# famoreno/stereo-vo

Hardware: AMD Instinct MI355X
Metric: stereo pairs/sec @1280×960 (higher is better)
Workload: dtype u8/f64

## Files before the change

### stereo_vo_amd/csrc/k_detect.hip

```cpp
#include <algorithm>
#include "svo_device.h"
#include "svo_kernels.h"
#include "faster_dyn.hpp"
#include "../../include/svo_orb_tables.h"

__constant__ int c_umax[16];
__device__ __attribute__((aligned(16))) float4 g_brief_patf[SVO_BRIEF_NPAIRS];
__device__ __attribute__((aligned(16))) uint4 g_blur_gh[3 * 64], g_blur_gv[3 * 64];
#define SVO_DISC_E 256
__device__ uint32_t g_disc_m[SVO_DISC_E], g_disc_x[SVO_DISC_E];
#define DP_REACH SVO_BRIEF_REACH
#define DP_BW (2 * DP_REACH + 1)
#define DP_RW (DP_BW + 6)
#define DP_X0 (DP_REACH + 5)

hipError_t svo_upload_tables()
{
    hipError_t e = hipMemcpyToSymbol(HIP_SYMBOL(c_umax), svo_umax, sizeof(svo_umax));
    if (e != hipSuccess) return e;
    {
        static float4 pf[SVO_BRIEF_NPAIRS];
        for (int i = 0; i < SVO_BRIEF_NPAIRS; i++) pf[i] = make_float4((float)svo_brief_pat[i][0], (float)svo_brief_pat[i][2], (float)svo_brief_pat[i][1], (float)svo_brief_pat[i][3]);
        e = hipMemcpyToSymbol(HIP_SYMBOL(g_brief_patf), pf, sizeof(pf));
        if (e != hipSuccess) return e;
// ... 829 lines not shown
    return a;
}

__device__ __forceinline__ void sincos_f32(float x, float& sn, float& cs)
{
    const int k = (int)(x * 0.63661977f + 0.5f);
    const float fk = (float)k;
    const float r = ((x - fk * 1.5703125f) - fk * 4.837512969970703125e-4f) - fk * 7.54978995489188216e-8f;
    const float z = r * r;
    const float sp = ((-1.9515295891e-4f * z + 8.3321608736e-3f) * z - 1.6666654611e-1f) * z * r + r;
    const float cp = ((2.443315711809948e-5f * z - 1.388731625493765e-3f) * z + 4.166664568298827e-2f) * z * z - 0.5f * z + 1.0f;
    const bool odd = k & 1;
    const float s0 = odd ? cp : sp, c0 = odd ? sp : cp;
    sn = (k & 2) ? -s0 : s0;
    cs = (((k + 1) & 2) != 0) ? -c0 : c0;
}

__device__ __forceinline__ uint32_t udot4(uint32_t a, uint32_t b, uint32_t acc)
{
    return __builtin_amdgcn_udot4(a, b, acc, false);
}

template <int NW, bool TL>
__global__ void __launch_bounds__(NW * 64) k_describe(DevCtx c, FastDiv gx_div, int pre, int kpw)
{
    SVO_TL_SCOPE(c, TL_DESCRIBE, pre);
    __shared__ __attribute__((aligned(16))) uint32_t raw32[NW][2][DP_LROWS * DP_PW + 4];
    __shared__ __attribute__((aligned(16))) float4 s_pat[SVO_BRIEF_NPAIRS];
    __shared__ uint32_t s_disc_m[SVO_DISC_E], s_disc_x[SVO_DISC_E];
    static_assert(NW * 64 == SVO_BRIEF_NPAIRS && NW * 64 == SVO_DISC_E, "one table entry per thread");
    __shared__ __attribute__((aligned(16))) uint4 s_gh[TL ? 3 * 64 : 1], s_gv[TL ? 3 * 64 : 1];
    if (c.idle.w[0] | c.idle.w[1]) {
        const int img_b = c.debug_mode == DBG_LINEAR_TILES ? (int)(blockIdx.x / gx_div.d) : (int)(fastdiv(blockIdx.x >> 3, gx_div) * 8 + (blockIdx.x & 7));
        if (img_b < c.n_img && lane_idle(c, img_b >> 1)) return;
    }
    s_pat[threadIdx.x] = g_brief_patf[threadIdx.x]; s_disc_m[threadIdx.x] = g_disc_m[threadIdx.x]; s_disc_x[threadIdx.x] = g_disc_x[threadIdx.x];
    if (TL && threadIdx.x < 3 * 64) { s_gh[threadIdx.x] = g_blur_gh[threadIdx.x]; s_gv[threadIdx.x] = g_blur_gv[threadIdx.x]; }
    __syncthreads();
    const int wid = __builtin_amdgcn_readfirstlane((int)(threadIdx.x >> 6)), lane = threadIdx.x & 63;
    int img, bx;
    if (c.debug_mode == DBG_LINEAR_TILES) { img = blockIdx.x / gx_div.d; bx = blockIdx.x - img * gx_div.d; }
    else { const uint32_t r = blockIdx.x >> 3, grp = fastdiv(r, gx_div); bx = (int)(r - grp * gx_div.d); img = (int)(grp * 8 + (blockIdx.x & 7)); }
    if (img >= c.n_img) return;
    const int lane_id = img >> 1, vl0 = lane_id * c.oct_cap;
    const int n_end = __builtin_amdgcn_readfirstlane(pre ? c.desc_n[img] : c.n_slots);
    const int slot0 = (bx * NW + wid) * kpw;
    if (slot0 >= n_end) return;
    const int slot1 = min(slot0 + kpw, n_end);
    const long long fo0 = pre ? feat_base(c, vl0, 1 - c.lane[lane_id].prev_slot, img & 1) : 0;
    dp_v4i GH[3], GV[3];
#pragma unroll
    for (int t = 0; t < 3; t++) { if (!TL) { GH[t] = *(const dp_v4i*)&g_blur_gh[t * 64 + lane]; GV[t] = *(const dp_v4i*)&g_blur_gv[t * 64 + lane]; } else { GH[t] = dp_v4i{0, 0, 0, 0}; GV[t] = GH[t]; } }
#pragma unroll
    for (int t = 0; t < 3; t++) if (!TL) asm volatile("" : "+v"(GH[t]), "+v"(GV[t]));
    uint32_t w_pos = 0, w_lvl = 0;
    if (slot0 + lane < slot1) {
        if (pre) { const uint2 w = c.desc_work[(long long)img * c.raw_cap + slot0 + lane]; w_pos = w.x; w_lvl = w.y; }
        else w_pos = c.lvl_pos[(long long)img * c.raw_cap + slot0 + lane];
    }
    asm volatile("" : "+v"(w_pos), "+v"(w_lvl));
    auto item = [&](int slot, int& live, int& x, int& y, int& level) {
        const uint32_t pos = (uint32_t)__builtin_amdgcn_readlane((int)w_pos, slot - slot0);
        int lv = 0, ok = 1;
        if (pre) lv = __builtin_amdgcn_readlane((int)w_lvl, slot - slot0);
        else {
#pragma unroll
            for (int l = 1; l < SVO_MAX_LEVELS; l++) if (l < c.n_levels && slot >= c.lv[l].slot_off) lv = l;
            lv = __builtin_amdgcn_readfirstlane(lv);
            ok = __builtin_amdgcn_readfirstlane(slot - c.lv[lv].slot_off < c.lvl_n[img * SVO_MAX_LEVELS + lv] ? 1 : 0);
        }
        level = lv; live = ok; x = (int)(pos & 0xFFFFu); y = (int)(pos >> 16);
    };
    const uint8_t* base0; const uint8_t* pyr0 = c.pyr + (long long)img * c.pyr_bytes;
    {
        const uint64_t b = (uint64_t)(uintptr_t)c.img0[img];
        base0 = (const uint8_t*)(uintptr_t)(((uint64_t)(uint32_t)__builtin_amdgcn_readfirstlane((int)(b >> 32)) << 32) | (uint32_t)__builtin_amdgcn_readfirstlane((int)(uint32_t)b));
    }
    const int cr0 = (lane * 171) >> 9, cq0 = lane - 3 * cr0, cr1 = ((lane + 64) * 171) >> 9, cq1 = lane + 64 - 3 * cr1;
    auto stage = [&](uint32_t* dst, int x, int y, int level) {
        const int pitch = level == 0 ? c.img0_pitch : c.lv[level].pitch;
        const uint8_t* lim = level == 0 ? base0 : pyr0 + c.lv[level].offset;
        const uint8_t* org = lim + (uint32_t)((y - (DP_REACH + 3)) * pitch + (x - DP_X0));
        const uint32_t lb = (uint32_t)__builtin_amdgcn_readfirstlane((int)(uint32_t)(uintptr_t)(__attribute__((address_space(3))) uint32_t*)dst);
        glds16_asm(org + (uint32_t)(cr0 * pitch + 16 * cq0), lb);
        glds16_asm(org + (uint32_t)(cr1 * pitch + 16 * cq1), lb + 1024);
        if (lane < DP_RW * 3 - 128) glds16_asm(org + (uint32_t)(42 * pitch + 32), lb + 2048);
    };
    static_assert(DP_RW * 3 - 128 == 1, "the third DMA instruction carries chunk 128 alone");
    int live, x, y, level;
    item(slot0, live, x, y, level);
    if (live) stage(raw32[wid][0], x, y, level);
    const int n16 = lane & 15, q4 = lane >> 4;
    for (int slot = slot0; slot < slot1; slot++) {
        uint32_t* R32 = raw32[wid][(slot - slot0) & 1];
        int live_n = 0, x_n = 0, y_n = 0, level_n = 0;
        if (slot + 1 < slot1) item(slot + 1, live_n, x_n, y_n, level_n);
        live_n = __builtin_amdgcn_readfirstlane(live_n); x_n = __builtin_amdgcn_readfirstlane(x_n); y_n = __builtin_amdgcn_readfirstlane(y_n); level_n = __builtin_amdgcn_readfirstlane(level_n);
        asm volatile("s_waitcnt vmcnt(0)" ::: "memory");
        wave_lds_sync();
        if (live_n) stage(raw32[wid][(slot - slot0 + 1) & 1], x_n, y_n, level_n);
        if (live) {
            uint32_t m10u = 0; int m01 = 0, msum = 0;
#pragma unroll
            for (int i = 0; i < 4; i++) {
                const int en = i * 64 + lane;
                const int vr = en >> 3, d = en & 7;
                const uint32_t px = R32[(vr + 6) * DP_PW + 2 + d];
                const uint32_t s = udot4(px, s_disc_m[en], 0u);
                m10u = udot4(px, s_disc_x[en], m10u);
                msum += (int)s;
                m01 += __mul24(vr - 15, (int)s);
            }
            const int m10 = wave_sum_uniform((int)m10u - 15 * msum);
            m01 = wave_sum_uniform(m01);
            float angle, sn, cs;
            if (c.debug_mode == DBG_DESCRIBE_NO_TRIG) { angle = (float)(m10 & 255); sn = (float)(m01 & 255) * 0.001f; cs = 1.f - sn; }
            else { angle = atan2_deg((float)m01, (float)m10); sincos_f32(angle * 0.017453292f, sn, cs); }
            dp_v4i S[3][3];
            {
                if (TL) {
#pragma unroll
                    for (int t = 0; t < 3; t++) GH[t] = *(const dp_v4i*)&s_gh[t * 64 + lane];
                }
// ... 38 lines not shown
                        asm("v_sat_pk_u8_i16 %0, %1" : "=v"(s23) : "v"(h23));
                        *(uint32_t*)&Bl[(16 * ot + n16) * (4 * DP_PW) + 16 * nt + 4 * q4] = __builtin_amdgcn_perm(s23, s01, 0x05040100u);
                    }
                }
            }
            wave_lds_sync();
            const float MX = 12582912.0f + (float)(DP_REACH + (int)((uint8_t*)R32 - (uint8_t*)&raw32[0][0][0])), MY = 12582912.0f + (float)DP_REACH;
            const uint8_t* lds0 = (const uint8_t*)&raw32[0][0][0];
            unsigned long long bits[4];
            typedef float dp_f2 __attribute__((ext_vector_type(2)));
            const dp_f2 cs2 = { cs, cs }, sn2 = { sn, sn }, MX2 = { MX, MX }, MY2 = { MY, MY };
#pragma unroll
            for (int k = 0; k < 4; k++) {
                const float4 pt = s_pat[k * 64 + lane];
                const dp_f2 px = { pt.x, pt.y }, py = { pt.z, pt.w };
                const dp_f2 xs = (px * cs2 - py * sn2) + MX2, ys = (px * sn2 + py * cs2) + MY2;
                const uint32_t o0 = (__umul24(__float_as_uint(ys.x), 4 * DP_PW) + __float_as_uint(xs.x)) & 0xFFFFu;
                const uint32_t o1 = (__umul24(__float_as_uint(ys.y), 4 * DP_PW) + __float_as_uint(xs.y)) & 0xFFFFu;
                const int a = lds0[o0], b = lds0[o1];
                bits[k] = __ballot(a < b);
            }
            if (lane == 0) {
                if (pre) {
                    const long long fo = fo0 + slot;
                    unsigned long long* d = (unsigned long long*)(c.desc + fo * 32);
                    d[0] = bits[0]; d[1] = bits[1]; d[2] = bits[2]; d[3] = bits[3];
                    c.kps[fo].angle = angle;
                } else {
                    const LevelGeom& g = c.lv[level];
                    const long long o = (long long)img * c.raw_cap + slot;
                    unsigned long long* d = (unsigned long long*)(c.raw_desc + o * 32);
                    d[0] = bits[0]; d[1] = bits[1]; d[2] = bits[2]; d[3] = bits[3];
                    svo_keypoint k;
                    k.x = (float)x * g.scale; k.y = (float)y * g.scale; k.size = c.fast_orb ? 7.0f : 31.0f * g.scale; k.angle = angle;
                    k.response = c.lvl_resp[o]; k.octave = c.fast_orb ? 0 : level; k.class_id = -1;
                    c.raw_kps[o] = k;
                }
            }
        }
        live = live_n; x = x_n; y = y_n; level = level_n;
    }
}

typedef unsigned long long sad_row_t __attribute__((aligned(1)));
template <bool ANY_SLOT>
__device__ __forceinline__ void sad_patch_body(const DevCtx& c, int which)
{
    const int vs = blockIdx.y, vl = vs >> 1, side = vs & 1, lane_id = vl / c.oct_cap, oct = vl % c.oct_cap;
    if (oct >= c.n_oct || lane_idle(c, lane_id)) return;
    const int prev = c.lane[lane_id].prev_slot;
    const int cur = (ANY_SLOT && which) ? prev : 1 - prev;
    const int n = c.n_kps[feat_cnt_idx(vl, cur, side)];
    const int i = blockIdx.x * 32 + (threadIdx.x >> 3), r = threadIdx.x & 7;
    if (i >= n) return;
    const long long fo = feat_base(c, vl, cur, side) + i;
    const svo_keypoint k = c.kps[fo];
    const int W = c.ow[oct], H = c.oh[oct];
    const bool border = k.x < 3.0f || k.y < 3.0f || k.x > (float)(W - 5) || k.y > (float)(H - 5);
    if (ANY_SLOT && (k.x != k.x || k.y != k.y)) { if (r == 0) c.sad_flag[fo] = 1; return; }
    if (r == 0) c.sad_flag[fo] = border ? 1 : 0;
    if (border) return;
    int pitch;
    const uint8_t* img = level_ptr(c, lane_id * 2 + side, c.fast_orb ? oct : 0, pitch);
// ... 1100 lines not shown
    if (c.n_tiles <= 0) return;
    const long long total = (long long)c.n_tiles * c.n_img, unit = 8 * FT_CHUNK;
    hipLaunchKernelGGL(k_fast, dim3((unsigned)((total + unit - 1) / unit * unit)), dim3(FT_NT), 0, st, c);
}

template <class F> static auto select_form(int sel_max, F f)
{
    if (sel_max > 4096) return f(std::integral_constant<int, 8192>());
    if (sel_max > 2048) return f(std::integral_constant<int, 4096>());
    return f(std::integral_constant<int, 2048>());
}

void launch_select(const DevCtx& c, hipStream_t st)
{
    const dim3 grid(c.n_img, c.n_levels);
    auto select = [&](int pass) { select_form(c.sel_max, [&](auto s) { hipLaunchKernelGGL(k_select<decltype(s)::value>, grid, dim3(512), 0, st, c, pass); }); };
    select(0);
    hipLaunchKernelGGL(k_fast_redo, dim3(4096), dim3(FT_NT), 0, st, c);
    select(1);
    hipLaunchKernelGGL(k_harris, dim3(c.n_img, c.sel_max / 256, c.n_levels), dim3(256), 0, st, c);
    select_form(c.sel_max, [&](auto s) { constexpr int S = decltype(s)::value; hipLaunchKernelGGL(k_select_sort<S>, grid, dim3(512), (size_t)LdsSelectSort<S>{}.total(), st, c); });
}

void launch_describe(const DevCtx& c, const Knobs& k, int pre, hipStream_t st)
{
    if (c.n_slots <= 0) return;
    const int kpw = k.desc_kpw, per = 4 * kpw, gx = (c.n_slots + per - 1) / per, img8 = (c.n_img + 7) / 8 * 8;
    if (k.desc_tl) hipLaunchKernelGGL((k_describe<4, true>), dim3((unsigned)((long long)gx * img8)), dim3(256), 0, st, c, make_fastdiv((uint32_t)gx), (pre && !c.fast_orb) ? 1 : 0, kpw);
    else hipLaunchKernelGGL((k_describe<4, false>), dim3((unsigned)((long long)gx * img8)), dim3(256), 0, st, c, make_fastdiv((uint32_t)gx), (pre && !c.fast_orb) ? 1 : 0, kpw);
}

void launch_sad_patch(const DevCtx& c, hipStream_t st)
{
    const int n = c.fast_orb ? c.max_kps : std::min(c.n_slots, c.max_kps);
    if (n <= 0) return;
    hipLaunchKernelGGL(k_sad_patch, dim3((n + 31) / 32, c.n_lanes * c.oct_cap * 2), dim3(256), 0, st, c);
}

void launch_publish_img0(const DevCtx& c, const uint8_t* const* ptrs, hipStream_t st)
{
    ImgPtrs ip;
    for (int i = 0; i < 2 * SVO_MAX_LANES; i++) ip.p[i] = i < c.n_img ? ptrs[i] : nullptr;
    hipLaunchKernelGGL(k_publish_img0, dim3((c.n_img + 255) / 256), dim3(256), 0, st, c, ip);
}
void launch_sad_patch_slot(const DevCtx& c, int which, hipStream_t st)
{
    hipLaunchKernelGGL(k_sad_patch_slot, dim3((c.max_kps + 31) / 32, c.n_lanes * c.oct_cap * 2), dim3(256), 0, st, c, which);
}

template <class T> static LdsChunkedNms<typename T::Key> chunked_nms_layout(const DevCtx& c) { return {FO_PMAX, c.max_kps}; }
static int nms_pmax(const DevCtx& c)
{
// ... 102 lines not shown
```

### stereo_vo_amd/csrc/svo_api.hip

```cpp
#include "svo_device.h"
#include "svo_kernels.h"
#include "state_format.hpp"
#include "frame_call.hpp"
#include "lk_call.hpp"
#include "gftt_call.hpp"
#include "klt_call.hpp"
#include <math.h>
#include <string.h>
#include <stdio.h>
#include <stdlib.h>
#include <string>
#include <vector>
#include <mutex>
#include <map>
#include <memory>
#include <condition_variable>

#define HIPCHECK(expr) do { hipError_t _e = (expr); if (_e != hipSuccess) { ctx->last_error = std::string(#expr) + ": " + hipGetErrorString(_e); return SVO_ERR_HIP; } } while (0)

enum { KT_BEGIN, KT_RESIZE, KT_FAST, KT_SELECT, KT_DESCRIBE, KT_NMS, KT_HAM_LR, KT_LR_FILTER, KT_HAM_TRK, KT_TRK_FILTER,
       KT_RANSAC_HYP, KT_RANSAC_CNT, KT_TRK_FINAL, KT_GN, KT_RANSAC_HYP1, KT_RANSAC_CNT1, KT_RANSAC_HYP2, KT_RANSAC_CNT2,
       KT_SAD_PATCH, KT_LR_SAD, KT_TRK_SAD,
       KT_SELECT_8192, KT_NMS_16, KT_HAM_LR_WIDE, KT_HAM_TRK_WIDE, KT_TRK_FILTER_64,
       KT_EXPORT, KT_IMPORT, KT_EXPORT_WIN, KT_IMPORT_WIN,
// ... 32 lines not shown
        for (const char* name : { "librocprofiler-sdk-roctx.so.1", "librocprofiler-sdk-roctx.so", "libroctx64.so.4", "libroctx64.so" }) {
            void* h = dlopen(name, RTLD_LAZY | RTLD_GLOBAL);
            if (!h) continue;
            push = (int (*)(const char*))dlsym(h, "roctxRangePushA");
            pop = (int (*)())dlsym(h, "roctxRangePop");
            if (push && pop) return;
            push = nullptr; pop = nullptr;
        }
    }
};
RoctxApi& roctx_api() { static RoctxApi a; return a; }
struct Section {
    bool on;
    explicit Section(const char* name) : on(roctx_api().push != nullptr) { if (on) roctx_api().push(name); }
    ~Section() { if (on) roctx_api().pop(); }
    Section(const Section&) = delete; Section& operator=(const Section&) = delete;
};
}
extern "C" int svo_profiler_sections_enabled(void) { return roctx_api().push != nullptr; }

struct svo_ctx {
    svo_config cfg;
    Knobs knobs;
    svo_params params;
    int fast_th, orb_th;
    int klt_win;
    hipStream_t stream, stream0; bool own_stream;
    DevCtx dc;
    bool geom_ready, geom_once;
    int geom_w, geom_h, geom_nfe, geom_nlevels, geom_method, geom_noct;
    int raw_cap_alloc;
    uint8_t* d_img0; int img0_pitch_internal;
    uint8_t* d_img0_ring[2]; uint8_t* h_stage[2]; size_t slot_bytes;
    hipStream_t s_copy; hipEvent_t ev_h2d[2], ev_det[2]; bool ev_det_valid[2], ev_h2d_valid[2], up_ready; int up_slot, det_slot;
    long long pyr_bytes_alloc; int cand_total_alloc, rtab_alloc, tile_tab_alloc;
    std::vector<void*> allocs;
    std::string last_error;
    std::vector<TimedSpan> spans; std::vector<hipEvent_t> free_events;
    double kt_total[KT_EVERY]; long long kt_calls[KT_EVERY]; unsigned long long kt_mask;
    unsigned* d_ham_out; uint8_t* d_ham_q, *d_ham_t; int ham_cap_q, ham_cap_t;
    uint8_t* d_lk_pyr; size_t lk_pyr_cap; LkJobDev* d_lk_jobs; int lk_jobs_cap;
    float2* d_lk_pts, *d_lk_init, *d_lk_out; uint8_t* d_lk_status; float* d_lk_err; int lk_pts_cap;
    std::vector<LkJobDev> lk_jobs; bool lk_used;
    float* d_gftt_map; size_t gftt_map_cap; uint8_t* d_gftt_img; size_t gftt_img_cap; GfttJobDev* d_gftt_jobs; int gftt_jobs_cap;
    unsigned long long* d_gftt_keys; int* d_gftt_items; uint8_t* d_gftt_state; int* d_gftt_info;
    float2* d_gftt_seeds; int gftt_seeds_cap; float2* d_gftt_pts; float* d_gftt_resp; int gftt_pts_cap;
// ... 267 lines not shown
    ctx->d_lk_pyr = nullptr; ctx->lk_pyr_cap = 0; ctx->d_lk_jobs = nullptr; ctx->lk_jobs_cap = 0; ctx->lk_pts_cap = 0; ctx->lk_used = false;
    ctx->d_lk_pts = ctx->d_lk_init = ctx->d_lk_out = nullptr; ctx->d_lk_status = nullptr; ctx->d_lk_err = nullptr;
    ctx->d_gftt_map = nullptr; ctx->gftt_map_cap = 0; ctx->d_gftt_img = nullptr; ctx->gftt_img_cap = 0; ctx->d_gftt_jobs = nullptr; ctx->gftt_jobs_cap = 0;
    ctx->d_gftt_keys = nullptr; ctx->d_gftt_items = nullptr; ctx->d_gftt_state = nullptr; ctx->d_gftt_info = nullptr;
    ctx->d_gftt_seeds = nullptr; ctx->gftt_seeds_cap = 0; ctx->d_gftt_pts = nullptr; ctx->d_gftt_resp = nullptr; ctx->gftt_pts_cap = 0; ctx->gftt_used = false;
    memset(&ctx->klt, 0, sizeof(ctx->klt)); ctx->params_set = false; ctx->frame_parallel = false; ctx->ransac_feed_used = false;
    ctx->d_src = nullptr; ctx->src_pitch = 0; ctx->d_map_ptrs = nullptr; ctx->map_w = ctx->map_h = ctx->n_maps = 0;
    ctx->map_shared[0] = ctx->map_shared[1] = nullptr; ctx->d_rect_models = nullptr;
    memset(&ctx->imported, 0, sizeof(ctx->imported)); ctx->graph_replays = 0; ctx->capturing = false; ctx->frame_active_set = false; memset(&ctx->frame_active, 0, sizeof(ctx->frame_active)); ctx->use_graphs = false; ctx->d_anms = nullptr; ctx->post_event = nullptr; ctx->pose_cov = false; ctx->d_cov = nullptr; ctx->d_cov_mask = nullptr;
    ctx->landmarks = false; ctx->lmk_std = 1.0; ctx->d_lmk = nullptr; ctx->d_lmk_info = nullptr; ctx->d_lmk_cnt = nullptr;
    ctx->sad.cur.assign((size_t)cfg->n_lanes, 1); ctx->sad.prev.assign((size_t)cfg->n_lanes, 1); ctx->sad.drop.assign((size_t)cfg->n_lanes, 0);
    ctx->cip_ready = false; ctx->d_vals = nullptr; ctx->h_vals = nullptr; ctx->vals_bytes = 0;
    ctx->up_ready = false; ctx->up_slot = 0; ctx->det_slot = -1; ctx->s_copy = nullptr; ctx->slot_bytes = 0;
    for (int i = 0; i < 2; i++) { ctx->d_img0_ring[i] = nullptr; ctx->h_stage[i] = nullptr; ctx->ev_det_valid[i] = ctx->ev_h2d_valid[i] = false; }
    for (int i = 0; i < KT_EVERY; i++) { ctx->kt_total[i] = 0; ctx->kt_calls[i] = 0; }
    ctx->kt_mask = ~0ull;
    *out = ctx;
    knobs_read(&ctx->knobs, knobs_env);
    if (svo_ab_form_requested(ctx->knobs) && !svo_ab_kernels_built()) {
        ctx->last_error = "SVO_HAM_FP4=0 / SVO_DEBUG_MODE=14 / 52 ask for an A/B kernel form that this library was built without: load libsvo_hip_ab.so (SVO_HIP_LIB) or build with -DSVO_AB_KERNELS";
        return SVO_ERR_UNSUPPORTED;
    }
    HIPCHECK(hipSetDevice(cfg->device));
    if (cfg->stream) { ctx->stream = (hipStream_t)cfg->stream; ctx->own_stream = false; }
    else { HIPCHECK(hipStreamCreateWithFlags(&ctx->stream, hipStreamNonBlocking)); ctx->own_stream = true; }
    ctx->stream0 = ctx->stream;
    HIPCHECK(svo_upload_tables());
    DevCtx& d = ctx->dc;
    memset(&d, 0, sizeof(d));
    const int L = cfg->n_lanes, NI = 2 * L, MK = cfg->max_kps;
    const int OC = cfg->max_octaves < 1 ? 1 : (cfg->max_octaves > SVO_MAX_OCTAVES ? SVO_MAX_OCTAVES : cfg->max_octaves);
    const int NV = L * OC;
    d.n_lanes = L; d.n_img = NI; d.max_kps = MK; d.n_levels = SVO_MAX_LEVELS; d.oct_cap = OC; d.n_oct = 1; d.max_h = cfg->max_h;
    ctx->raw_cap_alloc = 2 * MK;
    ctx->pyr_bytes_alloc = pyramid_bytes(cfg->max_w, cfg->max_h, SVO_MAX_LEVELS);
    ctx->cand_total_alloc = (int)((long long)cfg->max_cand * 33 / 10) + 8 * 1024;
    ctx->rtab_alloc = 2 * (cfg->max_w + cfg->max_h) * SVO_MAX_LEVELS;
    ctx->img0_pitch_internal = align_up(cfg->max_w, 64);
    HIPCHECK(dev_alloc(ctx, &ctx->d_img0, (size_t)NI * ctx->img0_pitch_internal * cfg->max_h));
    HIPCHECK(dev_alloc(ctx, (uint8_t***)&d.img0, (size_t)NI));
    HIPCHECK(dev_alloc(ctx, &d.pyr, (size_t)NI * ctx->pyr_bytes_alloc));
    HIPCHECK(dev_alloc(ctx, &d.rtab, (size_t)ctx->rtab_alloc));
    ctx->tile_tab_alloc = 4 * ((cfg->max_w / SVO_FT_W + 2) * (cfg->max_h / SVO_FT_H + 2)) + 64;
    HIPCHECK(dev_alloc(ctx, (uint4**)&d.fast_tiles, (size_t)ctx->tile_tab_alloc));
    HIPCHECK(dev_alloc(ctx, &d.cand_keys, (size_t)NI * ctx->cand_total_alloc));
    HIPCHECK(dev_alloc(ctx, &d.cand_cnt, (size_t)NI * SVO_MAX_LEVELS * SVO_CNT_STRIDE));
// ... 1003 lines not shown
{
    DevCtx& d = ctx->dc; const svo_params& p = ctx->params;
    if (call.faster) {
        { Span s(ctx, KT_RESIZE); for (int l = 1; l < d.n_levels; l++) launch_half(d, l, st); }
        if (call.faster_anms) {
            if (ctx->dyn_fast) { Span s(ctx, KT_FASTER); launch_faster_dyn(d, ctx->d_cand64, ctx->d_fstats, ctx->dyn_target, ctx->klt_win, st); }
            else { Span s(ctx, KT_FASTER); launch_faster(d, ctx->d_cand64, p.initial_FAST_threshold, ctx->klt_win, st); }
            { Span s(ctx, KT_FASTER_NMS); launch_faster_anms(d, ctx->d_cand64, ctx->d_fanms, ctx->dyn_fast ? ctx->d_fstats : nullptr, ctx->dyn_target, st); }
            return;
        }
        if (ctx->dyn_fast) {
            { Span s(ctx, KT_FASTER); launch_faster_dyn(d, ctx->d_cand64, ctx->d_fstats, ctx->dyn_target, ctx->klt_win, st); }
            { Span s(ctx, KT_FASTER_NMS); launch_faster_nms_dyn(d, ctx->d_cand64, p.non_maximal_suppression, p.min_distance, ctx->d_fstats, ctx->dyn_target, st); }
            return;
        }
        { Span s(ctx, KT_FASTER); launch_faster(d, ctx->d_cand64, p.initial_FAST_threshold, ctx->klt_win, st); }
        { Span s(ctx, KT_FASTER_NMS); launch_faster_nms(d, ctx->d_cand64, p.non_maximal_suppression, p.min_distance, st); }
    } else if (d.fast_orb) {
        { Span s(ctx, KT_RESIZE); for (int l = 1; l < d.n_levels; l++) launch_half(d, l, st); }
        { Span s(ctx, KT_FAST); launch_fast(d, st); }
        if (p.non_maximal_suppression && p.nmsMethod == SVO_NMS_ADAPTIVE) {
            Span s(ctx, KT_SELECT); launch_fastorb_anms(d, ctx->d_anms, st);
        } else { Span s(ctx, KT_SELECT); launch_fastorb_nms(d, p.non_maximal_suppression, p.min_distance, st); }
        { Span s(ctx, KT_DESCRIBE); launch_describe(d, ctx->knobs, 0, st); }
    } else {
        { Span s(ctx, KT_RESIZE); for (int l = 1; l < d.n_levels; l++) launch_resize(d, l, st); }
        { Span s(ctx, KT_FAST); launch_fast(d, st); }
        if (!call.select_in_post) { Span s(ctx, kt_select(d)); launch_select(d, st); }
        if (d.debug_mode == DBG_DESCRIBE_BEFORE_NMS) { Span s(ctx, KT_DESCRIBE); launch_describe(d, ctx->knobs, 0, st); }
    }
}
static void enqueue_detect_post(svo_ctx* ctx, const FrameCall& call, hipStream_t st)
{
    DevCtx& d = ctx->dc; const svo_params& p = ctx->params;
    if (call.select_in_post && !d.fast_orb) { Span s(ctx, kt_select(d)); launch_select(d, st); }
    const bool described = d.fast_orb || d.debug_mode == DBG_DESCRIBE_BEFORE_NMS;
    { Span s(ctx, kt_nms(d)); launch_nms_rowsort(d, ctx->knobs, d.fast_orb ? call.nms_mode_oct : call.nms_mode, p.min_distance, described ? 0 : 1, st); }
    if (!described) { Span s(ctx, KT_DESCRIBE); launch_describe(d, ctx->knobs, 1, st); }
}
static void enqueue_match(svo_ctx* ctx, const FrameCall& call, hipStream_t st)
{
    DevCtx& d = ctx->dc; const svo_params& p = ctx->params;
    Section sec("_stg3"), sec2("stg3.find_pairings");
    if (p.match_method == SVO_SM_DESC_BF) {
        { Span s(ctx, wide_lists(d) ? KT_HAM_LR_WIDE : KT_HAM_LR); launch_hamming(d, ctx->knobs, 0, hamming_splits(ctx), st); }
        { Span s(ctx, KT_LR_FILTER); launch_match_lr_filter(d, p.enable_robust_1to1_match, p.max_y_diff, st); }
    } else if (p.match_method == SVO_SM_DESC_RBR) {
        Span s(ctx, KT_LR_FILTER);
        launch_match_lr_rbr(d, false, p.enable_robust_1to1_match, p.max_y_diff, call.minresp, (int)(size_t)p.orb_max_distance, st);
    } else {
        Span s(ctx, KT_LR_SAD);
        launch_match_lr_rbr(d, true, p.enable_robust_1to1_match, p.max_y_diff, call.minresp, call.max_sad_match, st);
    }
}
static void set_ransac_chunks(svo_ctx* ctx)
{
    DevCtx& d = ctx->dc;
    const int forced = ctx->knobs.rs_c0;
    d.rs_c0 = forced ? forced : (d.n_lanes * d.n_oct > 8 ? SVO_RANSAC_CHUNK0 : SVO_RANSAC_FEW);
    d.rs_c1 = d.rs_c0 > SVO_RANSAC_CHUNK1 ? d.rs_c0 : SVO_RANSAC_CHUNK1;
}
// ... 1678 lines not shown
```

### stereo_vo_amd/csrc/svo_kernels.h

```cpp
#pragma once
#include "svo_device.h"
#include "rectify_model.hpp"

struct GNParams {
    int use_robust_kernel, max_iters, initial_max_iters, max_incr_cost;
    int use_previous_pose_as_initial, use_custom_initial_pose;
    int min_distance, img_w, img_h;
    int pmax;
    int standalone;
    int pad;
    double kernel_param, min_mod_out_vector, residual_threshold;
    double init[6];
    uint8_t* mask_out;
};

bool svo_ab_kernels_built();
hipError_t svo_upload_tables();
hipError_t svo_raise_dyn_smem(const void* kernel, size_t bytes);
struct PrepArgs {
    const uint8_t* src[2 * SVO_MAX_LANES];
    const uint2* const* maps;
    uint8_t* dst; long long dst_img_stride; int dst_pitch;
    long long src_stride; int channels, w, h;
    LaneMask idle;
};
void launch_prepare(const PrepArgs& a, int n_img, hipStream_t st);
struct RectifyImage { RectifyModel m; uint2* dst; };
void launch_rectify_map(const RectifyImage* d_models, int n_img, int w, int h, hipStream_t st);
size_t handover_record_bytes(const DevCtx& c);
size_t handover_record_bytes(const DevCtx& c, bool windows);
void launch_export_frame(const DevCtx& c, uint8_t* blob, const LaneMask& win_cur, const LaneMask& win_prev, hipStream_t st);
void launch_import_frame(const DevCtx& c, const uint8_t* blob, size_t blob_bytes, int need_windows, hipStream_t st);
void launch_pack_values(const DevCtx& c, int lane, int which, int octave, uint8_t* dst, hipStream_t st);
void launch_begin_frame(const DevCtx& c, const uint8_t* const* ptrs, unsigned flags, const LaneMask& drop_prev, hipStream_t st);
void launch_resize(const DevCtx& c, int level, hipStream_t st);
void launch_fast(const DevCtx& c, hipStream_t st);
void launch_select(const DevCtx& c, hipStream_t st);
void launch_describe(const DevCtx& c, const Knobs& k, int pre, hipStream_t st);
void launch_sad_patch(const DevCtx& c, hipStream_t st);
void launch_publish_img0(const DevCtx& c, const uint8_t* const* ptrs, hipStream_t st);
void launch_sad_patch_slot(const DevCtx& c, int which, hipStream_t st);
hipError_t configure_nms_rowsort(const DevCtx& c);
size_t nms_rowsort_scratch_bytes(int n_img, int oct_cap, int n_keys);
int nms_rowsort_items(const DevCtx& c);
void launch_nms_rowsort(const DevCtx& c, const Knobs& k, int do_nms, int min_distance, int pre, hipStream_t st);
void launch_half(const DevCtx& c, int level, hipStream_t st);
void launch_fastorb_anms(const DevCtx& c, uint32_t* scratch3, hipStream_t st);
size_t fastorb_anms_scratch_words(int n_img, int cand_total);
void launch_fastorb_nms(const DevCtx& c, int do_nms, int min_distance, hipStream_t st);
void launch_faster(const DevCtx& c, unsigned long long* cand64, int fast_th, int klt_win, hipStream_t st);
hipError_t configure_faster_nms(const DevCtx& c);
void launch_faster_nms(const DevCtx& c, const unsigned long long* cand64, int do_nms, int min_distance, hipStream_t st);
void launch_faster_dyn(const DevCtx& c, unsigned long long* cand64, const svo_faster_stats* stats, double target, int klt_win, hipStream_t st);
void launch_faster_nms_dyn(const DevCtx& c, const unsigned long long* cand64, int do_nms, int min_distance, svo_faster_stats* stats, double target, hipStream_t st);
hipError_t configure_faster_anms(int max_kps);
size_t faster_anms_scratch_words(int n_img, int cand_total);
int faster_anms_max_candidates();
void launch_faster_anms(const DevCtx& c, const unsigned long long* cand64, unsigned long long* scratch, svo_faster_stats* stats, double target, hipStream_t st);
void launch_anms_list(const unsigned long long* keys, int n, int w, int h, int actual, int max_kps, unsigned long long* scratch, int n_cap, uint32_t* out_pos, hipStream_t st);
void launch_hamming(const DevCtx& c, const Knobs& k, int mode, int nsplit, hipStream_t st);
void launch_match_lr_filter(const DevCtx& c, int one_to_one, double max_y_diff, hipStream_t st);
// ... 105 lines not shown
```

### stereo_vo_amd/csrc/svo_knobs.cpp

```cpp
#include "svo_knobs.hpp"
#include <stdio.h>
#include <stdlib.h>

const char* knobs_env(const char* name) { return getenv(name); }

void knobs_read(Knobs* k, const char* (*get)(const char*))
{
    const auto num = [&](const char* name) { const char* e = get(name); return e ? atoi(e) : 0; };
    const auto zero = [&](const char* name) { const char* e = get(name); return e && atoi(e) == 0; };
    k->debug_mode = num("SVO_DEBUG_MODE");
    k->rest_prio = num("SVO_REST_PRIO") & 3;
    { const char* e = get("SVO_TIMELINE"); k->timeline = e && e[0] == '1'; }
    k->ham_fp4 = !zero("SVO_HAM_FP4");
    { const int v = num("SVO_HAM_SPLITS"); k->ham_splits = v > 0 ? v : 0; }
    k->copy_prio_normal = zero("SVO_COPY_PRIO");
    { const int v = num("SVO_RS_C0"); k->rs_c0 = (v == SVO_RANSAC_CHUNK0 || v == SVO_RANSAC_CHUNK1 || v == SVO_RANSAC_FEW) ? v : 0; }
    k->rc_split[0] = RC16_NSPLIT0; k->rc_split[1] = k->rc_split[2] = 1;
    if (const char* e = get("SVO_RC_SPLIT")) {
        int v[3] = { 0, 0, 0 };
        const int n = sscanf(e, "%d,%d,%d", &v[0], &v[1], &v[2]);
        for (int i = 0; i < 3; i++) { const int x = i < n ? v[i] : (n > 0 ? v[n - 1] : 0); if (x >= 1 && x <= 8) k->rc_split[i] = x; }
    }
    { const int v = num("SVO_GN_NT"); k->gn_nt = (v == 256 || v == 384 || v == 512) ? v : 384; }
    { const int v = num("SVO_DESC_KPW"); k->desc_kpw = (v >= 1 && v <= 64) ? v : 8; }
    k->desc_tl = !zero("SVO_DESC_TL");
    k->nms_nt = num("SVO_NMS_NT");
}
```

### stereo_vo_amd/csrc/svo_knobs.hpp

```cpp
#pragma once

enum DebugMode : int {
    DBG_NONE = 0,
    DBG_FAST_STOP_STAGED = 1,
    DBG_FAST_STOP_COMPACTED = 2,
    DBG_FAST_STOP_SCORED = 3,
    DBG_FAST_NO_PUBLISH = 4,
    DBG_RESIZE_NO_STAGING = 5,
    DBG_RESIZE_NO_BLEND = 6,
    DBG_RESIZE_NO_STORE = 7,
    DBG_LINEAR_TILES = 8,
    DBG_DESCRIBE_BEFORE_NMS = 9,
    DBG_GN_STOP_SETUP = 10,
    DBG_GN_ONE_ITER = 11,
    DBG_NO_SPEC_FAST_TH = 12,
    DBG_RC_REPLAY_ALL = 13,
    DBG_RC_VALU16 = 14,
    DBG_RC_NO_EARLY_STOP = 16,
    DBG_NMS_STOP_KEYS = 21,
    DBG_NMS_STOP_SORT = 22,
    DBG_NMS_STOP_GRID = 23,
    DBG_NMS_STOP_ACCEPT = 24,
    DBG_NMS_STOP_ROWSORT = 25,
    DBG_NMS_STOP_CELLS = 26,
// ... 31 lines not shown
{
    return dbg_in(m, DBG_FAST_STOP_STAGED, DBG_RESIZE_NO_STORE) || m == DBG_GN_STOP_SETUP || m == DBG_GN_ONE_ITER || dbg_in(m, DBG_NMS_STOP_KEYS, DBG_NMS_STOP_CELLS) ||
           m == DBG_SELECT_STOP_HIST || dbg_in(m, DBG_SSORT_STOP_RANGE, DBG_DESCRIBE_NO_TRIG) || dbg_in(m, DBG_GN_NO_TRACK_LOOP, DBG_GN_STOP_TRIANGULATE);
}

#define SVO_RANSAC_CHUNK0 32
#define SVO_RANSAC_FEW 320
#ifndef SVO_RANSAC_CHUNK1
#define SVO_RANSAC_CHUNK1 160
#endif
#define RC16_NSPLIT0 1

struct Knobs {
    int debug_mode;
    int rest_prio;
    bool timeline;
    bool ham_fp4;
    int ham_splits;
    bool copy_prio_normal;
    int rs_c0;
    int rc_split[3];
    int gn_nt;
    int desc_kpw;
    bool desc_tl;
    int nms_nt;
};

void knobs_read(Knobs* k, const char* (*get)(const char*));
const char* knobs_env(const char* name);

inline bool svo_ab_form_requested(const Knobs& k) { return !k.ham_fp4 || debug_mode_is_ab_form(k.debug_mode); }
```

Measured before the change: 74090.

## Make describe kernel persistent with compacted per-image work table

Replaces the fixed image×tile grid of the describe kernel with a persistent grid sized to a few blocks per CU. Each wave walks a prefix-sum table of per-image work chunks (skipping idle lanes and empty slots) and prefetches the next chunk's keypoints while processing the current one. This removes the many early-exit blocks that previously launched for images with few keypoints and improves load balance. It also pins waves-per-EU occupancy hints, at the cost of more scalar bookkeeping and inline-asm scalar loads.

```diff
diff --git a/stereo_vo_amd/csrc/k_detect.hip b/stereo_vo_amd/csrc/k_detect.hip
--- a/stereo_vo_amd/csrc/k_detect.hip
+++ b/stereo_vo_amd/csrc/k_detect.hip
@@ -875,7 +875,7 @@
 }
 
 template <int NW, bool TL>
-__global__ void __launch_bounds__(NW * 64) k_describe(DevCtx c, FastDiv gx_div, int pre, int kpw)
+__global__ void __launch_bounds__(NW * 64) __attribute__((amdgpu_waves_per_eu(TL ? 5 : 4, TL ? 5 : 4))) k_describe(DevCtx c, FastDiv kpw_div, int pre, int kpw)
 {
     SVO_TL_SCOPE(c, TL_DESCRIBE, pre);
     __shared__ __attribute__((aligned(16))) uint32_t raw32[NW][2][DP_LROWS * DP_PW + 4];
@@ -883,56 +883,82 @@
     __shared__ uint32_t s_disc_m[SVO_DISC_E], s_disc_x[SVO_DISC_E];
     static_assert(NW * 64 == SVO_BRIEF_NPAIRS && NW * 64 == SVO_DISC_E, "one table entry per thread");
     __shared__ __attribute__((aligned(16))) uint4 s_gh[TL ? 3 * 64 : 1], s_gv[TL ? 3 * 64 : 1];
-    if (c.idle.w[0] | c.idle.w[1]) {
-        const int img_b = c.debug_mode == DBG_LINEAR_TILES ? (int)(blockIdx.x / gx_div.d) : (int)(fastdiv(blockIdx.x >> 3, gx_div) * 8 + (blockIdx.x & 7));
-        if (img_b < c.n_img && lane_idle(c, img_b >> 1)) return;
-    }
     s_pat[threadIdx.x] = g_brief_patf[threadIdx.x]; s_disc_m[threadIdx.x] = g_disc_m[threadIdx.x]; s_disc_x[threadIdx.x] = g_disc_x[threadIdx.x];
     if (TL && threadIdx.x < 3 * 64) { s_gh[threadIdx.x] = g_blur_gh[threadIdx.x]; s_gv[threadIdx.x] = g_blur_gv[threadIdx.x]; }
     __syncthreads();
     const int wid = __builtin_amdgcn_readfirstlane((int)(threadIdx.x >> 6)), lane = threadIdx.x & 63;
-    int img, bx;
-    if (c.debug_mode == DBG_LINEAR_TILES) { img = blockIdx.x / gx_div.d; bx = blockIdx.x - img * gx_div.d; }
-    else { const uint32_t r = blockIdx.x >> 3, grp = fastdiv(r, gx_div); bx = (int)(r - grp * gx_div.d); img = (int)(grp * 8 + (blockIdx.x & 7)); }
-    if (img >= c.n_img) return;
-    const int lane_id = img >> 1, vl0 = lane_id * c.oct_cap;
-    const int n_end = __builtin_amdgcn_readfirstlane(pre ? c.desc_n[img] : c.n_slots);
-    const int slot0 = (bx * NW + wid) * kpw;
-    if (slot0 >= n_end) return;
-    const int slot1 = min(slot0 + kpw, n_end);
-    const long long fo0 = pre ? feat_base(c, vl0, 1 - c.lane[lane_id].prev_slot, img & 1) : 0;
+    const bool linear = c.debug_mode == DBG_LINEAR_TILES;
+    const int x8 = (int)(blockIdx.x & 7);
+    const int W = (int)(linear ? gridDim.x : gridDim.x >> 3) * NW;
+    const int n_tab = linear ? c.n_img : (c.n_img + 7) >> 3;
+    int tgt = (int)(linear ? blockIdx.x : blockIdx.x >> 3) * NW + wid;
+    int tab_n = 0, tab_p = 0, page = 0, page_base = 0, g = 0, before = 0;
+    auto load_tab = [&]() {
+        const int i = page * 64 + lane, im = linear ? i : i * 8 + x8;
+        int n = 0;
+        if (i < n_tab && im < c.n_img && !lane_idle(c, im >> 1)) n = pre ? c.desc_n[im] : c.n_slots;
+        const int m = (int)fastdiv((uint32_t)(n + kpw - 1), kpw_div);
+        tab_n = n; tab_p = 0;
+        const int cnt = min(64, n_tab - page * 64);
+        for (int t = 0; t < cnt; t++) { const int mt = __builtin_amdgcn_readlane(m, t); if (lane >= t) tab_p += mt; }
+    };
+    load_tab();
+    auto sload32 = [](const int* ptr) { int v; asm volatile("s_nop 4\n\ts_load_dword %0, %1, 0x0\n\ts_waitcnt lgkmcnt(0)" : "=s"(v) : "s"(ptr) : "memory"); return v; };
+    auto sload64 = [](const void* ptr) { uint64_t v; asm volatile("s_nop 4\n\ts_load_dwordx2 %0, %1, 0x0\n\ts_waitcnt lgkmcnt(0)" : "=s"(v) : "s"(ptr) : "memory"); return v; };
+    auto find = [&](int& img, int& s0, int& s1, uint64_t& base, int& o0) -> bool {
+        for (;;) {
+            if (g >= min(64, n_tab - page * 64)) {
+                if ((page + 1) * 64 >= n_tab) return false;
+                page++; page_base = before; g = 0;
+                load_tab();
+                continue;
+            }
+            const int end = page_base + __builtin_amdgcn_readlane(tab_p, g);
+            if (tgt < end) break;
+            before = end; g++;
+        }
+        const int i = page * 64 + g, im = linear ? i : i * 8 + x8, a = (tgt - before) * kpw;
+        img = im; s0 = a; s1 = min(a + kpw, __builtin_amdgcn_readlane(tab_n, g)); base = sload64(c.img0 + im); tgt += W;
+        o0 = pre ? (int)feat_base(c, (im >> 1) * c.oct_cap, 1 - sload32(&c.lane[im >> 1].prev_slot), im & 1) : im * c.raw_cap;
+        return true;
+    };
     dp_v4i GH[3], GV[3];
 #pragma unroll
     for (int t = 0; t < 3; t++) { if (!TL) { GH[t] = *(const dp_v4i*)&g_blur_gh[t * 64 + lane]; GV[t] = *(const dp_v4i*)&g_blur_gv[t * 64 + lane]; } else { GH[t] = dp_v4i{0, 0, 0, 0}; GV[t] = GH[t]; } }
 #pragma unroll
     for (int t = 0; t < 3; t++) if (!TL) asm volatile("" : "+v"(GH[t]), "+v"(GV[t]));
-    uint32_t w_pos = 0, w_lvl = 0;
-    if (slot0 + lane < slot1) {
-        if (pre) { const uint2 w = c.desc_work[(long long)img * c.raw_cap + slot0 + lane]; w_pos = w.x; w_lvl = w.y; }
-        else w_pos = c.lvl_pos[(long long)img * c.raw_cap + slot0 + lane];
-    }
-    asm volatile("" : "+v"(w_pos), "+v"(w_lvl));
+    auto fetch = [&](int img, int s0, int s1, uint32_t& w_pos, uint32_t& w_lvl) {
+        const long long i = (long long)img * c.raw_cap + min(s0 + lane, s1 - 1);
+        if (pre) { const uint2 w = c.desc_work[i]; w_pos = w.x; w_lvl = w.y; }
+        else { w_lvl = 0; w_pos = c.lvl_pos[i]; }
+    };
+    int img = 0, slot0 = 0, slot1 = 0, out0 = 0, nx_img = 0, nx_s0 = 0, nx_s1 = 0, nx_out0 = 0;
+    uint64_t base0 = 0, nx_base = 0;
+    uint32_t w_pos = 0, w_lvl = 0, nx_pos = 0, nx_lvl = 0;
+    if (!find(img, slot0, slot1, base0, out0)) return;
+    int p = slot0;
+    fetch(img, slot0, slot1, w_pos, w_lvl);
+    bool have_nx = find(nx_img, nx_s0, nx_s1, nx_base, nx_out0);
+    if (have_nx) fetch(nx_img, nx_s0, nx_s1, nx_pos, nx_lvl);
+    asm volatile("" : "+v"(w_pos), "+v"(w_lvl), "+v"(nx_pos), "+v"(nx_lvl));
     auto item = [&](int slot, int& live, int& x, int& y, int& level) {
         const uint32_t pos = (uint32_t)__builtin_amdgcn_readlane((int)w_pos, slot - slot0);
         int lv = 0, ok = 1;
         if (pre) lv = __builtin_amdgcn_readlane((int)w_lvl, slot - slot0);
         else {
-#pragma unroll
-            for (int l = 1; l < SVO_MAX_LEVELS; l++) if (l < c.n_levels && slot >= c.lv[l].slot_off) lv = l;
+            int lv_mask = (1 << c.n_levels) - 1;
+            asm volatile("" : "+s"(lv_mask));
+#pragma unroll
+            for (int l = 1; l < SVO_MAX_LEVELS; l++) if (((lv_mask >> l) & 1) && slot >= c.lv[l].slot_off) lv = l;
             lv = __builtin_amdgcn_readfirstlane(lv);
             ok = __builtin_amdgcn_readfirstlane(slot - c.lv[lv].slot_off < c.lvl_n[img * SVO_MAX_LEVELS + lv] ? 1 : 0);
         }
         level = lv; live = ok; x = (int)(pos & 0xFFFFu); y = (int)(pos >> 16);
     };
-    const uint8_t* base0; const uint8_t* pyr0 = c.pyr + (long long)img * c.pyr_bytes;
-    {
-        const uint64_t b = (uint64_t)(uintptr_t)c.img0[img];
-        base0 = (const uint8_t*)(uintptr_t)(((uint64_t)(uint32_t)__builtin_amdgcn_readfirstlane((int)(b >> 32)) << 32) | (uint32_t)__builtin_amdgcn_readfirstlane((int)(uint32_t)b));
-    }
     const int cr0 = (lane * 171) >> 9, cq0 = lane - 3 * cr0, cr1 = ((lane + 64) * 171) >> 9, cq1 = lane + 64 - 3 * cr1;
     auto stage = [&](uint32_t* dst, int x, int y, int level) {
         const int pitch = level == 0 ? c.img0_pitch : c.lv[level].pitch;
-        const uint8_t* lim = level == 0 ? base0 : pyr0 + c.lv[level].offset;
+        const uint8_t* lim = level == 0 ? (const uint8_t*)(uintptr_t)base0 : c.pyr + (long long)img * c.pyr_bytes + c.lv[level].offset;
         const uint8_t* org = lim + (uint32_t)((y - (DP_REACH + 3)) * pitch + (x - DP_X0));
         const uint32_t lb = (uint32_t)__builtin_amdgcn_readfirstlane((int)(uint32_t)(uintptr_t)(__attribute__((address_space(3))) uint32_t*)dst);
         glds16_asm(org + (uint32_t)(cr0 * pitch + 16 * cq0), lb);
@@ -941,17 +967,28 @@
     };
     static_assert(DP_RW * 3 - 128 == 1, "the third DMA instruction carries chunk 128 alone");
     int live, x, y, level;
-    item(slot0, live, x, y, level);
+    item(p, live, x, y, level);
+    int out = out0 + p++;
     if (live) stage(raw32[wid][0], x, y, level);
     const int n16 = lane & 15, q4 = lane >> 4;
-    for (int slot = slot0; slot < slot1; slot++) {
-        uint32_t* R32 = raw32[wid][(slot - slot0) & 1];
-        int live_n = 0, x_n = 0, y_n = 0, level_n = 0;
-        if (slot + 1 < slot1) item(slot + 1, live_n, x_n, y_n, level_n);
+    for (int buf = 0, more = 1; more; buf ^= 1) {
+        uint32_t* R32 = raw32[wid][buf];
+        int live_n = 0, x_n = 0, y_n = 0, level_n = 0, refill = 0;
+        int out_n = 0;
+        if (p >= slot1) {
+            more = have_nx ? 1 : 0;
+            if (more) { img = nx_img; slot0 = nx_s0; slot1 = nx_s1; base0 = nx_base; out0 = nx_out0; w_pos = nx_pos; w_lvl = nx_lvl; p = slot0; refill = 1; }
+        }
+        if (more) { item(p, live_n, x_n, y_n, level_n); out_n = out0 + p++; }
         live_n = __builtin_amdgcn_readfirstlane(live_n); x_n = __builtin_amdgcn_readfirstlane(x_n); y_n = __builtin_amdgcn_readfirstlane(y_n); level_n = __builtin_amdgcn_readfirstlane(level_n);
         asm volatile("s_waitcnt vmcnt(0)" ::: "memory");
+        asm volatile("" : "+v"(nx_pos), "+v"(nx_lvl));
         wave_lds_sync();
-        if (live_n) stage(raw32[wid][(slot - slot0 + 1) & 1], x_n, y_n, level_n);
+        if (live_n) stage(raw32[wid][buf ^ 1], x_n, y_n, level_n);
+        if (refill) {
+            have_nx = find(nx_img, nx_s0, nx_s1, nx_base, nx_out0);
+            if (have_nx) fetch(nx_img, nx_s0, nx_s1, nx_pos, nx_lvl);
+        }
         if (live) {
             uint32_t m10u = 0; int m01 = 0, msum = 0;
 #pragma unroll
@@ -1036,13 +1073,13 @@
             }
             if (lane == 0) {
                 if (pre) {
-                    const long long fo = fo0 + slot;
+                    const long long fo = out;
                     unsigned long long* d = (unsigned long long*)(c.desc + fo * 32);
                     d[0] = bits[0]; d[1] = bits[1]; d[2] = bits[2]; d[3] = bits[3];
                     c.kps[fo].angle = angle;
                 } else {
                     const LevelGeom& g = c.lv[level];
-                    const long long o = (long long)img * c.raw_cap + slot;
+                    const long long o = out;
                     unsigned long long* d = (unsigned long long*)(c.raw_desc + o * 32);
                     d[0] = bits[0]; d[1] = bits[1]; d[2] = bits[2]; d[3] = bits[3];
                     svo_keypoint k;
@@ -1052,7 +1089,7 @@
                 }
             }
         }
-        live = live_n; x = x_n; y = y_n; level = level_n;
+        live = live_n; x = x_n; y = y_n; level = level_n; out = out_n;
     }
 }
 
@@ -2199,12 +2236,20 @@
     select_form(c.sel_max, [&](auto s) { constexpr int S = decltype(s)::value; hipLaunchKernelGGL(k_select_sort<S>, grid, dim3(512), (size_t)LdsSelectSort<S>{}.total(), st, c); });
 }
 
-void launch_describe(const DevCtx& c, const Knobs& k, int pre, hipStream_t st)
+static int describe_grid(int n_slots, int n_img, int kpw, int bpc, int n_cu)
+{
+    const int gx = (n_slots + kpw - 1) / kpw, img8 = (n_img + 7) / 8 * 8;
+    const long long cap = (long long)((gx + 3) / 4) * img8, want = (long long)bpc * n_cu / 8 * 8;
+    return (int)std::max(8ll, std::min(cap, want));
+}
+
+void launch_describe(const DevCtx& c, const Knobs& k, int n_cu, int pre, hipStream_t st)
 {
     if (c.n_slots <= 0) return;
-    const int kpw = k.desc_kpw, per = 4 * kpw, gx = (c.n_slots + per - 1) / per, img8 = (c.n_img + 7) / 8 * 8;
-    if (k.desc_tl) hipLaunchKernelGGL((k_describe<4, true>), dim3((unsigned)((long long)gx * img8)), dim3(256), 0, st, c, make_fastdiv((uint32_t)gx), (pre && !c.fast_orb) ? 1 : 0, kpw);
-    else hipLaunchKernelGGL((k_describe<4, false>), dim3((unsigned)((long long)gx * img8)), dim3(256), 0, st, c, make_fastdiv((uint32_t)gx), (pre && !c.fast_orb) ? 1 : 0, kpw);
+    const int kpw = k.desc_kpw;
+    const dim3 grid((unsigned)describe_grid(c.n_slots, c.n_img, kpw, k.desc_bpc, n_cu));
+    if (k.desc_tl) hipLaunchKernelGGL((k_describe<4, true>), grid, dim3(256), 0, st, c, make_fastdiv((uint32_t)kpw), (pre && !c.fast_orb) ? 1 : 0, kpw);
+    else hipLaunchKernelGGL((k_describe<4, false>), grid, dim3(256), 0, st, c, make_fastdiv((uint32_t)kpw), (pre && !c.fast_orb) ? 1 : 0, kpw);
 }
 
 void launch_sad_patch(const DevCtx& c, hipStream_t st)
diff --git a/stereo_vo_amd/csrc/svo_api.hip b/stereo_vo_amd/csrc/svo_api.hip
--- a/stereo_vo_amd/csrc/svo_api.hip
+++ b/stereo_vo_amd/csrc/svo_api.hip
@@ -78,6 +78,7 @@
 struct svo_ctx {
     svo_config cfg;
     Knobs knobs;
+    int n_cu;
     svo_params params;
     int fast_th, orb_th;
     int klt_win;
@@ -391,6 +392,7 @@
         return SVO_ERR_UNSUPPORTED;
     }
     HIPCHECK(hipSetDevice(cfg->device));
+    HIPCHECK(hipDeviceGetAttribute(&ctx->n_cu, hipDeviceAttributeMultiprocessorCount, cfg->device));
     if (cfg->stream) { ctx->stream = (hipStream_t)cfg->stream; ctx->own_stream = false; }
     else { HIPCHECK(hipStreamCreateWithFlags(&ctx->stream, hipStreamNonBlocking)); ctx->own_stream = true; }
     ctx->stream0 = ctx->stream;
@@ -1440,12 +1442,12 @@
         if (p.non_maximal_suppression && p.nmsMethod == SVO_NMS_ADAPTIVE) {
             Span s(ctx, KT_SELECT); launch_fastorb_anms(d, ctx->d_anms, st);
         } else { Span s(ctx, KT_SELECT); launch_fastorb_nms(d, p.non_maximal_suppression, p.min_distance, st); }
-        { Span s(ctx, KT_DESCRIBE); launch_describe(d, ctx->knobs, 0, st); }
+        { Span s(ctx, KT_DESCRIBE); launch_describe(d, ctx->knobs, ctx->n_cu, 0, st); }
     } else {
         { Span s(ctx, KT_RESIZE); for (int l = 1; l < d.n_levels; l++) launch_resize(d, l, st); }
         { Span s(ctx, KT_FAST); launch_fast(d, st); }
         if (!call.select_in_post) { Span s(ctx, kt_select(d)); launch_select(d, st); }
-        if (d.debug_mode == DBG_DESCRIBE_BEFORE_NMS) { Span s(ctx, KT_DESCRIBE); launch_describe(d, ctx->knobs, 0, st); }
+        if (d.debug_mode == DBG_DESCRIBE_BEFORE_NMS) { Span s(ctx, KT_DESCRIBE); launch_describe(d, ctx->knobs, ctx->n_cu, 0, st); }
     }
 }
 static void enqueue_detect_post(svo_ctx* ctx, const FrameCall& call, hipStream_t st)
@@ -1454,7 +1456,7 @@
     if (call.select_in_post && !d.fast_orb) { Span s(ctx, kt_select(d)); launch_select(d, st); }
     const bool described = d.fast_orb || d.debug_mode == DBG_DESCRIBE_BEFORE_NMS;
     { Span s(ctx, kt_nms(d)); launch_nms_rowsort(d, ctx->knobs, d.fast_orb ? call.nms_mode_oct : call.nms_mode, p.min_distance, described ? 0 : 1, st); }
-    if (!described) { Span s(ctx, KT_DESCRIBE); launch_describe(d, ctx->knobs, 1, st); }
+    if (!described) { Span s(ctx, KT_DESCRIBE); launch_describe(d, ctx->knobs, ctx->n_cu, 1, st); }
 }
 static void enqueue_match(svo_ctx* ctx, const FrameCall& call, hipStream_t st)
 {
diff --git a/stereo_vo_amd/csrc/svo_kernels.h b/stereo_vo_amd/csrc/svo_kernels.h
--- a/stereo_vo_amd/csrc/svo_kernels.h
+++ b/stereo_vo_amd/csrc/svo_kernels.h
@@ -36,7 +36,7 @@
 void launch_resize(const DevCtx& c, int level, hipStream_t st);
 void launch_fast(const DevCtx& c, hipStream_t st);
 void launch_select(const DevCtx& c, hipStream_t st);
-void launch_describe(const DevCtx& c, const Knobs& k, int pre, hipStream_t st);
+void launch_describe(const DevCtx& c, const Knobs& k, int n_cu, int pre, hipStream_t st);
 void launch_sad_patch(const DevCtx& c, hipStream_t st);
 void launch_publish_img0(const DevCtx& c, const uint8_t* const* ptrs, hipStream_t st);
 void launch_sad_patch_slot(const DevCtx& c, int which, hipStream_t st);
diff --git a/stereo_vo_amd/csrc/svo_knobs.cpp b/stereo_vo_amd/csrc/svo_knobs.cpp
--- a/stereo_vo_amd/csrc/svo_knobs.cpp
+++ b/stereo_vo_amd/csrc/svo_knobs.cpp
@@ -22,7 +22,13 @@
         for (int i = 0; i < 3; i++) { const int x = i < n ? v[i] : (n > 0 ? v[n - 1] : 0); if (x >= 1 && x <= 8) k->rc_split[i] = x; }
     }
     { const int v = num("SVO_GN_NT"); k->gn_nt = (v == 256 || v == 384 || v == 512) ? v : 384; }
-    { const int v = num("SVO_DESC_KPW"); k->desc_kpw = (v >= 1 && v <= 64) ? v : 8; }
+    k->desc_kpw = 8; k->desc_bpc = 3;
+    if (const char* e = get("SVO_DESC_KPW")) {
+        int v[2] = { 0, 0 };
+        sscanf(e, "%d,%d", &v[0], &v[1]);
+        if (v[0] >= 1 && v[0] <= 64) k->desc_kpw = v[0];
+        if (v[1] >= 1 && v[1] <= 5) k->desc_bpc = v[1];
+    }
     k->desc_tl = !zero("SVO_DESC_TL");
     k->nms_nt = num("SVO_NMS_NT");
 }
diff --git a/stereo_vo_amd/csrc/svo_knobs.hpp b/stereo_vo_amd/csrc/svo_knobs.hpp
--- a/stereo_vo_amd/csrc/svo_knobs.hpp
+++ b/stereo_vo_amd/csrc/svo_knobs.hpp
@@ -77,6 +77,7 @@
     int rc_split[3];
     int gn_nt;
     int desc_kpw;
+    int desc_bpc;
     bool desc_tl;
     int nms_nt;
 };
```

Measured after the change: 73090. -1.3%, worse.
